# DavidLBick/espnet-1

Measured on AMD Instinct MI355X. Metric: utterances/sec + step-time, Conformer-L T=1000 batch=32 @1/2/4/8 GPU, higher is better.
Workload: dtype bf16; 1 GPU; C3 Conformer-L (12x512, 8 heads, ff 2048, cnn 31) + 6-layer Transformer decoder, hybrid CTC/att 0.3/0.7, lsm 0.1, V=5000, T=1000 frames x 80, L=40, dropout 0.1, Adam+WarmupLR+clip 5; global_batch=32, seq_len=1000, parallelism=dp1

## Files before the change

espnet-1_amd/csrc/gemm.hip:

```cpp

#include "gemm_kern.h"
#include <cstdio>
#include <cstdlib>

namespace {
__global__ void splitk_reduce(GemmP p) {
  const long MN = (long)p.M * p.N;
  const int z = blockIdx.y;
  const int zb = z / p.nh, zh = z % p.nh;
  const float* base = p.ws + (long)z * p.splitk * MN;
  const bool vec = p.vec_c && (p.N % 4 == 0);
  const EpiK ek = make_epik(p);
  const long n4 = vec ? MN / 4 : MN;
  for (long i = blockIdx.x * (long)blockDim.x + threadIdx.x; i < n4; i += (long)gridDim.x * blockDim.x) {
    if (vec) {
      float4 a = make_float4(0.f, 0.f, 0.f, 0.f);
      int s = 0;
      for (; s + 8 <= p.splitk; s += 8) {
        float4 b[8];
#pragma unroll
        for (int j = 0; j < 8; ++j) b[j] = *(const float4*)(base + (long)(s + j) * MN + i * 4);
#pragma unroll
        for (int j = 0; j < 8; ++j) { a.x += b[j].x; a.y += b[j].y; a.z += b[j].z; a.w += b[j].w; }
      }
// ... 80 lines not shown
  EA_LAUNCH_CHECK();
  return 0;
}

}

extern "C" int ea_gemm_set_pipeline(int stages) {
  EA_ENTRY();
  EA_CHECK_ARG(stages == 0 || stages == 2 || stages == 12);
  g_gemm_bm64 = stages < 10;
  g_gemm_stages = stages % 10;
  return 0;
}

namespace {
__global__ void probe_begin_kernel(unsigned long long* s) { s[0] = ~0ull; s[1] = 0ull; }
__global__ void probe_end_kernel(unsigned long long* s) {
  if (s[1] > s[0]) { s[2] += s[1] - s[0]; s[3] += 1ull; }
}
}

namespace {
__global__ void phase_stamp_kernel(unsigned long long* st, float* ring, int cap, int phase, const float* extra,
                                   const int* skip) {
  const unsigned long long now = __builtin_amdgcn_s_memrealtime();
  if (phase > 0) {
    const long slot = (long)(st[1] % (unsigned long long)cap);
    float dt = (float)((double)(now - st[0]) * 1e-8);
    if (phase == 3 && skip && skip[0]) dt = __builtin_nanf("");
    ring[slot * 4 + phase - 1] = dt;
    if (phase == 3) {
      ring[slot * 4 + 3] = extra ? extra[0] : 0.f;
      st[1] = st[1] + 1ull;
    }
  }
  st[0] = now;
}
}

extern "C" int ea_phase_stamp(unsigned long long* state, float* ring, int cap, int phase, const float* extra,
                              void* stream) {
  EA_ENTRY();
  EA_CHECK_ARG(state != nullptr && ring != nullptr && cap > 0 && phase >= 0 && phase <= 3);
  hipLaunchKernelGGL(phase_stamp_kernel, dim3(1), dim3(1), 0, (hipStream_t)stream, state, ring, cap, phase, extra,
                     (const int*)nullptr);
  EA_LAUNCH_CHECK();
  return 0;
}

extern "C" int ea_phase_stamp_opt(unsigned long long* state, float* ring, int cap, int phase,
                                  const ea_opt_state* opt, void* stream) {
  EA_ENTRY();
  EA_CHECK_ARG(state != nullptr && ring != nullptr && cap > 0 && phase >= 0 && phase <= 3 && opt != nullptr);
  hipLaunchKernelGGL(phase_stamp_kernel, dim3(1), dim3(1), 0, (hipStream_t)stream, state, ring, cap, phase,
                     &opt->next_lr, &opt->skip);
  EA_LAUNCH_CHECK();
  return 0;
}

extern "C" int ea_gemm_set_diag(unsigned long long* buf) {
  EA_ENTRY();
  g_diag = buf;
  return 0;
}

extern "C" int ea_gemm_set_probe(unsigned long long* slots) {
  EA_ENTRY();
  g_probe = slots;
  return 0;
}

extern "C" int ea_probe_begin(unsigned long long* slots, void* stream) {
  EA_ENTRY();
  EA_CHECK_ARG(slots != nullptr);
  hipLaunchKernelGGL(probe_begin_kernel, dim3(1), dim3(1), 0, (hipStream_t)stream, slots);
  EA_LAUNCH_CHECK();
  return 0;
}

extern "C" int ea_probe_end(unsigned long long* slots, void* stream) {
  EA_ENTRY();
  EA_CHECK_ARG(slots != nullptr);
  hipLaunchKernelGGL(probe_end_kernel, dim3(1), dim3(1), 0, (hipStream_t)stream, slots);
  EA_LAUNCH_CHECK();
  return 0;
}

extern "C" int ea_gemm_set_pipe(int on) {
  EA_ENTRY();
  g_gemm_pipe = on;
  return 0;
}

extern "C" int ea_gemm_set_k128(int mode, int slots) {
  EA_ENTRY();
  EA_CHECK_ARG(mode >= 0 && mode <= 3 && (slots == 3 || slots == 4));
  g_gemm_k128 = mode;
  eag::g_k128_slots = slots;
  return 0;
}

extern "C" int ea_gemm_set_skinny(int max_m) {
  EA_ENTRY();
  EA_CHECK_ARG(max_m >= 0 && max_m <= 64);
  g_gemm_skinny = max_m;
  return 0;
}

extern "C" int ea_gemm_set_tile(int bm, int bn) {
  EA_ENTRY();
  EA_CHECK_ARG((bm == 0 && bn == 0) || (bm == 32 && bn == 128) || (bm == 64 && bn == 128) ||
               (bm == 128 && bn == 128) || (bm == 256 && bn == 256));
  g_force_bm = bm;
  g_force_bn = bn;
  return 0;
}

static int gemm_impl(int dtype, int a_kmajor, int b_kmajor, int M, int N, int K,
                     const void* A, long lda, long sAb, long sAh,
                     const void* B, long ldb, long sBb, long sBh,
                     int batch, int nh,
                     void* C, int c_dtype, long ldc, long sCb, long sCh,
                     const ea_epilogue* epi, float* workspace, long ws_elems, void* stream,
                     const ea_conv_geo* geo, const float* w1x = nullptr, int w1T = 0, int w1F = 0,
                     float* w1part = nullptr, const uint8_t* w1pos = nullptr) {
  EA_CHECK_ARG(epi != nullptr && M >= 0 && N >= 0 && K >= 0 && batch >= 1 && nh >= 1);
  EA_CHECK_ARG(dtype == EA_F32 || dtype == EA_BF16);
  if (M == 0 || N == 0) return 0;
  const int E = dtype == EA_BF16 ? 8 : 4;
  const int esz = dtype == EA_BF16 ? 2 : 4;
  (void)esz;
  if (epi->kind == EA_EPI_RESID) EA_CHECK_ARG(c_dtype == EA_F32);
  GemmP p{};
  p.M = M; p.N = N; p.K = K;
  p.A = A; p.lda = lda; p.sAb = sAb; p.sAh = sAh;
  p.B = B; p.ldb = ldb; p.sBb = sBb; p.sBh = sBh;
  p.nh = nh;
  p.C = C; p.c_dtype = c_dtype; p.ldc = ldc; p.sCb = sCb; p.sCh = sCh;
  p.epi = *epi;
  p.ws = workspace;
  p.salt = ea_g_rng_salt;
  p.stamp = g_probe;
  p.diag = g_diag;
  p.g = geo ? *geo : ea_conv_geo{};
  p.w1x = w1x; p.w1part = w1part; p.w1pos = w1pos; p.w1T = w1T; p.w1F = w1F;
  p.vec_a = (lda % E == 0 && sAb % E == 0 && sAh % E == 0 && ((uintptr_t)A % 16) == 0);
  p.vec_b = (ldb % E == 0 && sBb % E == 0 && sBh % E == 0 && ((uintptr_t)B % 16) == 0);
  {
    const int ce = c_dtype == EA_BF16 ? 2 : 4;
    bool vc = (N % 4 == 0) && ldc % 4 == 0 && sCb % 4 == 0 && sCh % 4 == 0 && ((uintptr_t)C % (4 * ce)) == 0;
    if (epi->bias) vc = vc && ((uintptr_t)epi->bias % 16) == 0;
    if (epi->aux) vc = vc && epi->ldaux % 4 == 0 && ((uintptr_t)epi->aux % (4 * (epi->aux_dtype == EA_BF16 ? 2 : 4))) == 0;
    if (epi->resid) vc = vc && epi->ldr % 4 == 0 && ((uintptr_t)epi->resid % 16) == 0;
    p.vec_c = vc;
    bool v8 = vc && N % 8 == 0 && ldc % 8 == 0 && sCb % 8 == 0 && sCh % 8 == 0 && ((uintptr_t)C % 16) == 0;
    if (epi->aux) v8 = v8 && epi->ldaux % 8 == 0 && ((uintptr_t)epi->aux % 16) == 0;
    if (epi->resid) v8 = v8 && epi->ldr % 8 == 0;
    p.vec8 = v8;
  }
  p.bm = 128; p.bn = 128;
  if (dtype == EA_BF16 && M <= g_gemm_skinny && a_kmajor && b_kmajor && !geo && !w1part &&
      batch * nh == 1 && K % 32 == 0 && K > 0 && p.vec_a && p.vec_b) {
    static const bool trace_s = std::getenv("EA_GEMM_TRACE") != nullptr;
    if (trace_s) std::fprintf(stderr, "[ea_gemm] M=%d N=%d K=%d skinny epi=%d\n", M, N, K, (int)epi->kind);
    return launch_skinny(p, (hipStream_t)stream);
  }
  const double a_ext = 2.0 * ((a_kmajor ? (double)M : (double)K) * lda);
  const double b_ext = 2.0 * ((b_kmajor ? (double)N : (double)K) * ldb);
  const bool lds_path = dtype == EA_BF16 && p.vec_a && p.vec_b && g_gemm_stages > 0 &&
                        a_ext < 4.0e9 && b_ext < 4.0e9;
  p.lds = lds_path;
  if (geo && geo->mode != 0) {
    if (!lds_path || K % 64 != 0 || geo->C % 64 != 0 || batch * nh != 1) return EA_ERR_BAD_ARG;
    if ((geo->mode == EA_CONV_WGRAD) == (a_kmajor != 0) || (geo->mode == EA_CONV_FWD) != (b_kmajor != 0))
      return EA_ERR_BAD_ARG;
    choose_tile(p, 0, 1);
    if (geo->mode == EA_CONV_WGRAD && !g_force_bm) { p.bm = 256; p.bn = 256; }
    if (w1part) {
      if (!g_gemm_pipe || !p.vec8) return EA_ERR_BAD_ARG;
      p.bm = 256; p.bn = 256;
    }
    if (p.bm != 256 || p.bn != 256) { p.bm = 128; p.bn = 128; }
  } else if (lds_path) {
    choose_tile(p, a_kmajor, (long)batch * nh);
  }
  bool k128 = false;
  if (g_gemm_k128 && lds_path && !geo && a_kmajor && b_kmajor && K % 64 == 0 && K > 0) {
    const long t128 = (long)ea_cdiv(M, 128) * ea_cdiv(N, 128) * batch * nh;
    const bool fits = g_gemm_k128 == 3 ||
                      (!g_force_bm && (p.bm == 64 || p.bm == 128) && p.bn == 128 && t128 >= 128 &&
                       (g_gemm_k128 == 2 || (t128 <= 256 && K >= 1024)));
    if (fits) { p.bm = 128; p.bn = 128; k128 = true; }
  }
  if (p.bm <= 64 && !a_kmajor) return EA_ERR_BAD_ARG;
  p.tiles_m = ea_cdiv(M, p.bm);
  p.tiles_n = ea_cdiv(N, p.bn);
  const int KT = dtype == EA_BF16 ? KCfg<bf16>::KT : KCfg<float>::KT;
  const int nz = batch * nh;
  int splitk = 1;
  const long tiles = max(1L, (long)p.tiles_m * p.tiles_n * nz * (p.bm * p.bn) / (128 * 128));
  if (geo && geo->mode == EA_CONV_WGRAD && p.bm == 256) {
    if (workspace) {
      splitk = max(1, 256 / (p.tiles_m * p.tiles_n));
      splitk = min(splitk, K / (4 * KT));
      while (splitk > 1 && (long)splitk * M * N > ws_elems) --splitk;
      splitk = max(splitk, 1);
    }
  } else if (!k128 && workspace && tiles < 200 && K >= 16 * KT && K >= 1024 && (long)p.tiles_m * p.tiles_n * nz < 128) {
    splitk = (int)((384 + tiles - 1) / tiles);
    splitk = min(splitk, K / (4 * KT));
    splitk = min(splitk, 16);
    while (splitk > 1 && (long)splitk * nz * M * N > ws_elems) --splitk;
    if (splitk < 1) splitk = 1;
  }
  int kchunk = K;
  if (splitk > 1) {
    kchunk = ea_cdiv(ea_cdiv(K, splitk), KT) * KT;
    splitk = ea_cdiv(K, kchunk);
  }
  p.splitk = splitk;
  p.kchunk = kchunk;
  static const bool trace = std::getenv("EA_GEMM_TRACE") != nullptr;
  if (trace)
    std::fprintf(stderr, "[ea_gemm] M=%d N=%d K=%d ak=%d bk=%d nz=%d tile=%dx%d%s splitk=%d epi=%d geo=%d lds=%d\n", M,
                 N, K, a_kmajor, b_kmajor, nz, p.bm, p.bn, k128 ? "k" : "", splitk, (int)epi->kind, geo ? geo->mode : 0,
                 (int)p.lds);
  hipStream_t st = (hipStream_t)stream;
  int rc = dtype == EA_BF16 ? launch<bf16>(p, a_kmajor, b_kmajor, nz, st, k128)
                            : launch<float>(p, a_kmajor, b_kmajor, nz, st);
  if (rc) return rc;
  if (splitk > 1) {
    const long MN = (long)M * N;
    dim3 grid(ea_grid_cap(ea_cdiv(MN / 4 + 1, 256), 2048), nz);
    hipLaunchKernelGGL(splitk_reduce, grid, dim3(256), 0, st, p);
    EA_LAUNCH_CHECK();
  }
  return 0;
}

extern "C" int ea_gemm(int dtype, int a_kmajor, int b_kmajor, int M, int N, int K,
                       const void* A, long lda, long sAb, long sAh,
                       const void* B, long ldb, long sBb, long sBh,
                       int batch, int nh,
                       void* C, int c_dtype, long ldc, long sCb, long sCh,
                       const ea_epilogue* epi, float* workspace, long ws_elems, void* stream) {
  EA_ENTRY();
  return gemm_impl(dtype, a_kmajor, b_kmajor, M, N, K, A, lda, sAb, sAh, B, ldb, sBb, sBh, batch, nh, C, c_dtype,
                   ldc, sCb, sCh, epi, workspace, ws_elems, stream, nullptr);
}

extern "C" int ea_gemm_ln(int M, int N, int K, const float* x, long ldx, const float* gamma, const float* beta,
                          float eps, const void* W, long ldw, void* C, int c_dtype, long ldc, const ea_epilogue* epi,
                          void* stream) {
  EA_ENTRY();
  EA_CHECK_ARG(epi != nullptr && M >= 0 && N >= 0 && K > 0 && K % 32 == 0 && K <= 32 * 8 * 8);
  EA_CHECK_ARG(x && gamma && beta && W && C && ldx >= K && ldw >= K && ldc >= N);
  EA_CHECK_ARG(ldx % 4 == 0 && ((uintptr_t)x % 16) == 0 && ldw % 8 == 0 && ((uintptr_t)W % 16) == 0 &&
               ((uintptr_t)gamma % 16) == 0 && ((uintptr_t)beta % 16) == 0);
  if (epi->kind == EA_EPI_RESID) EA_CHECK_ARG(c_dtype == EA_F32);
  if (M == 0 || N == 0) return 0;
  GemmP p{};
  p.M = M; p.N = N; p.K = K;
  p.A = x; p.lda = ldx;
  p.B = W; p.ldb = ldw;
  p.nh = 1; p.splitk = 1; p.kchunk = K;
  p.C = C; p.c_dtype = c_dtype; p.ldc = ldc;
  p.epi = *epi;
  p.salt = ea_g_rng_salt;
  const int ce = c_dtype == EA_BF16 ? 2 : 4;
  bool vc = (N % 4 == 0) && ldc % 4 == 0 && ((uintptr_t)C % (4 * ce)) == 0;
  if (epi->bias) vc = vc && ((uintptr_t)epi->bias % 16) == 0;
  if (epi->aux) vc = vc && epi->ldaux % 4 == 0 && ((uintptr_t)epi->aux % (4 * (epi->aux_dtype == EA_BF16 ? 2 : 4))) == 0;
  if (epi->resid) vc = vc && epi->ldr % 4 == 0 && ((uintptr_t)epi->resid % 16) == 0;
  p.vec_c = vc;
  return launch_skinny_ln(p, gamma, beta, eps, (hipStream_t)stream);
}

extern "C" int ea_gemm_conv(const ea_conv_geo* geo, int a_kmajor, int b_kmajor, int M, int N, int K,
                            const void* A, long lda, const void* B, long ldb, void* C, int c_dtype, long ldc,
                            const ea_epilogue* epi, float* workspace, long ws_elems, void* stream) {
  EA_ENTRY();
  EA_CHECK_ARG(geo != nullptr && geo->mode >= EA_CONV_FWD && geo->mode <= EA_CONV_WGRAD);
  return gemm_impl(EA_BF16, a_kmajor, b_kmajor, M, N, K, A, lda, 0, 0, B, ldb, 0, 0, 1, 1, C, c_dtype, ldc, 0, 0,
                   epi, workspace, ws_elems, stream, geo);
}

extern "C" int ea_gemm_conv_w1(const ea_conv_geo* geo, int M, int N, int K, const void* A, long lda, const void* B,
                               long ldb, const ea_epilogue* epi, const float* x, int T, int Fin, float* part,
                               void* stream) {
  EA_ENTRY();
  EA_CHECK_ARG(geo != nullptr && geo->mode == EA_CONV_DGRAD && x != nullptr && part != nullptr);
  EA_CHECK_ARG(epi != nullptr && epi->kind == EA_EPI_DACT && epi->act == EA_ACT_RELU && epi->aux != nullptr &&
               epi->aux_dtype == EA_BF16);
  EA_CHECK_ARG(T >= 3 && Fin >= 3 && M < (1 << 24));
  return gemm_impl(EA_BF16, 1, 0, M, N, K, A, lda, 0, 0, B, ldb, 0, 0, 1, 1, nullptr, EA_BF16, N, 0, 0, epi,
                   nullptr, 0, stream, geo, x, T, Fin, part);
}

extern "C" int ea_gemm_conv_w1b(const ea_conv_geo* geo, int M, int N, int K, const void* A, long lda, const void* B,
                                long ldb, const ea_epilogue* epi, const float* x, int T, int Fin, float* part,
                                const unsigned char* pos, void* stream) {
  EA_ENTRY();
  EA_CHECK_ARG(geo != nullptr && geo->mode == EA_CONV_DGRAD && x != nullptr && part != nullptr && pos != nullptr);
  EA_CHECK_ARG(epi != nullptr && epi->kind == EA_EPI_DACT && epi->act == EA_ACT_RELU && N % 8 == 0);
  EA_CHECK_ARG(T >= 3 && Fin >= 3 && M < (1 << 24));
  return gemm_impl(EA_BF16, 1, 0, M, N, K, A, lda, 0, 0, B, ldb, 0, 0, 1, 1, nullptr, EA_BF16, N, 0, 0, epi,
                   nullptr, 0, stream, geo, x, T, Fin, part, pos);
}


extern "C" int ea_gemm_conv_w1b_all(const ea_conv_geo* geo, int N, const void* A, long lda, const void* B, long ldb,
                                    const ea_epilogue* epi, const float* x, int T, int Fin, float* part,
                                    const unsigned char* pos, void* stream) {
  EA_ENTRY();
  EA_CHECK_ARG(geo != nullptr && geo->mode == EA_CONV_DGRAD && x != nullptr && part != nullptr && pos != nullptr);
  EA_CHECK_ARG(epi != nullptr && epi->kind == EA_EPI_DACT && epi->act == EA_ACT_RELU);
  EA_CHECK_ARG(N >= 8 && N % 8 == 0 && geo->C % 64 == 0 && T >= 3 && Fin >= 3 && g_gemm_pipe != 0);
  EA_CHECK_ARG(lda % 8 == 0 && ldb % 8 == 0 && ((uintptr_t)A % 16) == 0 && ((uintptr_t)B % 16) == 0);
  GemmP p{};
  p.N = N;
  p.A = A; p.lda = lda;
  p.B = B; p.ldb = ldb;
  p.nh = 1; p.splitk = 1;
  p.C = nullptr; p.c_dtype = EA_BF16; p.ldc = N;
  p.epi = *epi;
  p.salt = ea_g_rng_salt;
  p.stamp = g_probe;
  p.diag = g_diag;
  p.g = *geo;
  p.w1x = x; p.w1part = part; p.w1pos = pos; p.w1T = T; p.w1F = Fin;
  p.vec_a = p.vec_b = p.vec_c = p.vec8 = p.lds = 1;
  p.bm = p.bn = 256;
  p.tiles_n = ea_cdiv(N, 256);
  int items = 0, tiles = 0;
  for (int c = 0; c < 4; ++c) {
    const int a = c >> 1, e = c & 1;
    const long rows = (long)geo->B * geo->nI[a] * geo->nJ[e];
    EA_CHECK_ARG(rows < (1L << 24));
    if (rows == 0) continue;
    const int k = p.ncls++;
    p.cls_item0[k] = items;
    p.cls_M[k] = (int)rows;
    p.cls_K[k] = (a ? 1 : 2) * (e ? 1 : 2) * geo->C;
    p.cls_a[k] = a;
    p.cls_e[k] = e;
    p.cls_tile0[k] = tiles;
    p.cls_pos[k] = geo->plane[c] / geo->C * (N / 8);
    tiles += (int)ea_cdiv(rows, 256);
    items += (int)ea_cdiv(rows, 256) * p.tiles_n;
  }
  if (p.ncls == 0) return 0;
  p.cls_item0[p.ncls] = items;
  p.M = p.cls_M[0]; p.K = p.cls_K[0]; p.kchunk = p.K; p.tiles_m = ea_cdiv(p.M, 256);
  const int unit = 8 * p.tiles_n;
  const dim3 grid((unsigned)(ea_cdiv(items, unit) * unit));
  static const bool trace = std::getenv("EA_GEMM_TRACE") != nullptr;
  if (trace) std::fprintf(stderr, "[ea_gemm] conv dgrad x%d classes, %d tiles, grid %u\n", p.ncls, items, grid.x);
  return launch_pipe_conv(p, grid, (hipStream_t)stream);
}
```

espnet-1_amd/csrc/gemm_kern.h:

```cpp
#pragma once
#include "common.h"


namespace eag {

constexpr int BM = 128, BN = 128, NT = 256;
constexpr int TILE_BYTES = 16384;

template <typename T> struct KCfg;
template <> struct KCfg<bf16> { static constexpr int KT = 64, KS = 32, E = 8, NKS = 2; };
template <> struct KCfg<float> { static constexpr int KT = 32, KS = 4, E = 4, NKS = 8; };

struct GemmP {
  int M, N, K;
  const void* A; long lda, sAb, sAh;
  const void* B; long ldb, sBb, sBh;
  int nh, splitk, kchunk;
  void* C; int c_dtype; long ldc, sCb, sCh;
  ea_epilogue epi;
  float* ws;
  int tiles_m, tiles_n;
  int vec_a, vec_b;
  int vec_c;
  int vec8;
// ... 1109 lines not shown
    const int row = c >> 2, ch = c & 3;
    return row * 64 + ((ch ^ swz32(row)) << 4);
  } else {
    const int pnl = c >> 9, cj = c & 511, k = cj >> 4, ch = cj & 15;
    return pnl * 8192 + k * 256 + ((ch ^ swz_mn_bf16(k)) << 4);
  }
}

EA_DEV s16x4 tr_read_asm(const char* p) {
  s16x4 v;
  const uint32_t a = (uint32_t)(uintptr_t)(const __attribute__((address_space(3))) char*)p;
  asm volatile("ds_read_b64_tr_b16 %0, %1" : "=v"(v) : "v"(a) : "memory");
  return v;
}

template <bool KMAJ>
EA_DEV bf16x8 frag32(const char* img, int r, int lane) {
  if (KMAJ) {
    const int row = r + (lane & 15), ch = lane >> 4;
    return *(const bf16x8*)(img + row * 64 + ((ch ^ swz32(row)) << 4));
  }
  const char* pnl = img + (r >> 7) * 8192;
  const int i = lane & 15, q = i >> 2, pp = i & 3;
  const int col = (r & 127) + 4 * pp;
  const int ch = col >> 3, within = (col & 7) * 2;
  union { bf16x8 v; s16x4 h[2]; } out;
#pragma unroll
  for (int half = 0; half < 2; ++half) {
    const int row = 8 * (lane >> 4) + 4 * half + q;
    out.h[half] = tr_read_asm(pnl + row * 256 + ((ch ^ swz_mn_bf16(row)) << 4) + within);
  }
  return out.v;
}

template <int BT, int NS = 4>
struct PipeT {
  static constexpr int BK = 32, NSLOT = NS, NW = 8, NTT = 512;
  static constexpr int A_BYTES = BT * BK * 2, B_BYTES = BT * BK * 2, SLOT = A_BYTES + B_BYTES;
  static constexpr int RING = NSLOT * SLOT;
  static constexpr int MI = BT == 256 ? 8 : 2;
  static constexpr int EPI_BYTES = NW * (MI < 4 ? MI : 4) * 16 * EPI_LDT * 4;
  static constexpr int SMEM = RING > EPI_BYTES ? RING : EPI_BYTES;
  static constexpr int ACH = A_BYTES / (NTT * 16), BCH = B_BYTES / (NTT * 16);
  static constexpr int G = ACH + BCH;
  static constexpr int OCC = BT == 256 ? 1 : 2;
  static_assert(BT == 256 || BT == 128, "pipe tiles");
  static_assert(NS == 4, "ring depth: 4 slots (5- and 6/8-slot rings measured slower, round 3/4)");
  EA_DEV static int wm(int w) { return BT == 256 ? (w >> 2) * 128 : (w >> 2) * 64 + ((w >> 1) & 1) * 32; }
  EA_DEV static int wn(int w) { return BT == 256 ? (w & 3) * 64 : (w & 1) * 64; }
};

struct TileOv {
  int M, a, e;
  float* w1part;
  const uint8_t* w1pos;
};
EA_DEV TileOv tile_ov(const GemmP& p) { return TileOv{p.M, p.g.a, p.g.e, p.w1part, p.w1pos}; }

template <bool AK, bool BKM, int MODE = 0, int BT = 256, int NS = 4>
EA_DEV void pipe_tile(const GemmP& p, const TileOv& ov, char* smem, const bf16* A, const bf16* B, int m0, int n0, int kbeg,
                      int kend, f32x4 (&acc)[PipeT<BT, NS>::MI][4]) {
  static_assert(MODE == 0 || (MODE == EA_CONV_FWD && AK && BKM) || (MODE == EA_CONV_DGRAD && AK) ||
                (MODE == EA_CONV_WGRAD && !AK && !BKM), "conv gather layouts");
  static_assert(MODE == 0 || BT == 256, "conv gathers run on 256-wide tiles");
  using PC = PipeT<BT, NS>;
  constexpr int BK = PC::BK, NSLOT = PC::NSLOT, NW = PC::NW, NTT = PC::NTT, MI = PC::MI;
  constexpr int A_BYTES = PC::A_BYTES, B_BYTES = PC::B_BYTES, SLOT = PC::SLOT;
  constexpr int ACH = PC::ACH, BCH = PC::BCH, G = PC::G;
  const int tid = threadIdx.x, lane = tid & 63, w = tid >> 6;
  const int wm = PC::wm(w), wn = PC::wn(w);
  const int nsl = max(0, (kend - kbeg) / BK);
  const bool tail = kbeg + nsl * BK < kend;


  auto src = [&](long ld, int mn0, int MN, bool kmaj, int ci) -> uint32_t {
    if (kmaj) {
      const int row = ci >> 2, c = (ci & 3) ^ swz32(ci >> 2);
      return (uint32_t)(((long)min(mn0 + row, MN - 1) * ld + c * 8) * 2);
    }
    const int pnl = ci >> 9, cj = ci & 511, k = cj >> 4, c = (cj & 15) ^ swz_mn_bf16(k);
    return (uint32_t)(((long)k * ld + min((long)(mn0 + pnl * 128 + c * 8), (long)((MN - 1) & ~7))) * 2);
  };
  const char* abase = (const char*)(A + (AK ? (long)kbeg : (long)kbeg * p.lda));
  const char* bbase = (const char*)(B + (BKM ? (long)kbeg : (long)kbeg * p.ldb));
  uint32_t aoff[ACH], boff[BCH];
#pragma unroll
  for (int i = 0; i < ACH; ++i) aoff[i] = src(p.lda, m0, ov.M, AK, (i * NW + w) * 64 + lane);
#pragma unroll
  for (int i = 0; i < BCH; ++i) boff[i] = src(p.ldb, n0, p.N, BKM, (i * NW + w) * 64 + lane);
  const long astep = (AK ? BK : (long)BK * p.lda) * 2;
  const long bstep = (BKM ? BK : (long)BK * p.ldb) * 2;

  const int ksl0 = kbeg / BK;
  const int CS = MODE ? p.g.C / BK : 1;
  int gb[ACH], gt[ACH], gf[ACH], cur[ACH];
  if constexpr (MODE == EA_CONV_FWD || MODE == EA_CONV_DGRAD) {
    const int n2 = MODE == EA_CONV_FWD ? p.g.T2 : p.g.nI[ov.a];
    const int n3 = MODE == EA_CONV_FWD ? p.g.F2 : p.g.nJ[ov.e];
#pragma unroll
    for (int i = 0; i < ACH; ++i) {
      const int m = min(m0 + ((((i * NW + w) * 64 + lane)) >> 2), ov.M - 1);
      const int bt = fdiv(m, n3);
      gf[i] = m - bt * n3;
      gb[i] = fdiv(bt, n2);
      gt[i] = bt - gb[i] * n2;
      cur[i] = 0;
    }
  }
  auto a_tap = [&](int q) {
#pragma unroll
    for (int i = 0; i < ACH; ++i) {
      const int ci = (i * NW + w) * 64 + lane;
      const int cc = ((ci & 3) ^ swz32(ci >> 2)) * 8;
      if constexpr (MODE == EA_CONV_FWD) {
        const int kh = q / 3, kw = q - 3 * (q / 3);
        cur[i] = (int)x1p_row(p.g, gb[i], gt[i], gf[i], kh, kw) + cc;
      } else {
        int kh, kw;
        dgrad_tap2(ov.a, ov.e, q, kh, kw);
        const int t2 = gt[i] - (kh >> 1), f2 = gf[i] - (kw >> 1);
        cur[i] = (t2 >= 0 && t2 < p.g.T2 && f2 >= 0 && f2 < p.g.F2)
                     ? ((gb[i] * p.g.T2 + t2) * p.g.F2 + f2) * p.g.C + cc
                     : (int)p.g.zero + ((ci >> 2) & 63) * p.g.C + cc;
      }
    }
  };
  int wb[BCH], wt[BCH], wf[BCH], wpix[BCH], wbase[BCH], wnI[BCH], wnJ[BCH];
  if constexpr (MODE == EA_CONV_WGRAD) {
#pragma unroll
    for (int i = 0; i < BCH; ++i) {
      const int ci = (i * NW + w) * 64 + lane;
      const int pnl = ci >> 9, cj = ci & 511, k = cj >> 4, c = (cj & 15) ^ swz_mn_bf16(k);
      const int n = min(n0 + pnl * 128 + c * 8, p.N - 8);
      const int tap = n / p.g.C, cin = n - tap * p.g.C;
      const int kh = tap / 3, kw = tap - 3 * kh, a = kh & 1, e = kw & 1;
      wnI[i] = p.g.nI[a];
      wnJ[i] = p.g.nJ[e];
      wbase[i] = (int)p.g.plane[a * 2 + e] + ((kh >> 1) * wnJ[i] + (kw >> 1)) * p.g.C + cin;
      const int pix = ksl0 * BK + k;
      wpix[i] = pix;
      const int bt = fdiv(pix, p.g.F2);
      wf[i] = pix - bt * p.g.F2;
      wb[i] = fdiv(bt, p.g.T2);
      wt[i] = bt - wb[i] * p.g.T2;
    }
  }
  const int dF = BK % max(p.g.F2, 1), dT = BK / max(p.g.F2, 1);

  auto issue = [&](int sl) {
    char* base = smem + (sl % NSLOT) * SLOT;
    const char* ak = abase + sl * astep;
    const char* bk = bbase + sl * bstep;
    if constexpr (MODE == EA_CONV_FWD || MODE == EA_CONV_DGRAD) {
      const int ks = ksl0 + sl;
      int q, c0;
      bool newtap;
      if constexpr (MODE == EA_CONV_FWD) {
        const int cb = ks / 18, r = ks - 18 * cb;
        q = r >> 1;
        c0 = cb * 64 + (r & 1) * BK;
        newtap = (r & 1) == 0;
      } else {
        q = ks / CS;
        c0 = (ks - q * CS) * BK;
        newtap = c0 == 0;
      }
      if (newtap || sl == 0) a_tap(q);
#pragma unroll
      for (int i = 0; i < ACH; ++i)
        __builtin_amdgcn_global_load_lds((__attribute__((address_space(1))) void*)((const char*)A + (long)(cur[i] + c0) * 2),
                                         (__attribute__((address_space(3))) void*)(base + (i * NW + w) * 1024), 16, 0, 0);
      if constexpr (MODE == EA_CONV_DGRAD) {
        int kh, kw;
        dgrad_tap2(ov.a, ov.e, q, kh, kw);
        bk = BKM ? (const char*)(B + (long)(kh * 3 + kw) * p.g.C + c0)
                 : (const char*)(B + ((long)(kh * 3 + kw) * p.g.C + c0) * p.g.C);
      }
    } else {
#pragma unroll
      for (int i = 0; i < ACH; ++i)
        __builtin_amdgcn_global_load_lds((__attribute__((address_space(1))) void*)(ak + aoff[i]),
                                         (__attribute__((address_space(3))) void*)(base + (i * NW + w) * 1024), 16, 0, 0);
    }
    if constexpr (MODE == EA_CONV_WGRAD) {
#pragma unroll
      for (int i = 0; i < BCH; ++i) {
        const int off = wpix[i] < p.g.P ? wbase[i] + ((wb[i] * wnI[i] + wt[i]) * wnJ[i] + wf[i]) * p.g.C
                                        : (int)p.g.zero + (lane & 63) * p.g.C + (wbase[i] % p.g.C);
        __builtin_amdgcn_global_load_lds((__attribute__((address_space(1))) void*)((const char*)B + (long)off * 2),
                                         (__attribute__((address_space(3))) void*)(base + A_BYTES + (i * NW + w) * 1024),
                                         16, 0, 0);
        wpix[i] += BK;
        wf[i] += dF;
        wt[i] += dT;
        if (wf[i] >= p.g.F2) { wf[i] -= p.g.F2; ++wt[i]; }
        while (wt[i] >= p.g.T2) { wt[i] -= p.g.T2; ++wb[i]; }
      }
    } else {
#pragma unroll
      for (int i = 0; i < BCH; ++i)
        __builtin_amdgcn_global_load_lds((__attribute__((address_space(1))) void*)(bk + boff[i]),
                                         (__attribute__((address_space(3))) void*)(base + A_BYTES + (i * NW + w) * 1024),
                                         16, 0, 0);
    }
  };

  auto rd_b = [&](int sl, bf16x8 (&fb)[4]) {
    const char* lb = smem + (sl % NSLOT) * SLOT + A_BYTES;
#pragma unroll
    for (int j = 0; j < 4; ++j) fb[j] = frag32<BKM>(lb, wn + j * 16, lane);
  };
  auto rd_a = [&](int sl, bf16x8 (&fa)[MI]) {
    const char* la = smem + (sl % NSLOT) * SLOT;
#pragma unroll
    for (int i = 0; i < MI; ++i) fa[i] = frag32<AK>(la, wm + i * 16, lane);
  };

  const int g1 = w >> 2;
  const int npre = min(NSLOT - 1, nsl);
  for (int sl = 0; sl < npre; ++sl) issue(sl);
  wait_newer<G, NSLOT - 2>(npre - 1);
  lds_barrier();
  if (g1) lds_barrier();
  bf16x8 fa[MI], fb[4];
  for (int sl = 0; sl < nsl; ++sl) {
    __builtin_amdgcn_sched_barrier(0);
    rd_b(sl, fb);
    rd_a(sl, fa);
    if (sl + NSLOT - 1 < nsl) issue(sl + NSLOT - 1);
    wait_newer<G, NSLOT - 2>(min(NSLOT - 2, nsl - 2 - sl));
    if (!AK || !BKM) {
      asm volatile("s_waitcnt lgkmcnt(0)" ::: "memory");
      __builtin_amdgcn_sched_barrier(0);
    }
#pragma unroll
    for (int i = 0; i < MI; ++i) asm volatile("" ::"v"(fa[i]));
#pragma unroll
    for (int j = 0; j < 4; ++j) asm volatile("" ::"v"(fb[j]));
    __builtin_amdgcn_sched_barrier(0);
    lds_barrier();
    __builtin_amdgcn_sched_barrier(0);
    __builtin_amdgcn_s_setprio(1);
#pragma unroll
    for (int i = 0; i < MI; ++i)
#pragma unroll
      for (int j = 0; j < 4; ++j)
        acc[i][j] = __builtin_amdgcn_mfma_f32_16x16x32_bf16(fa[i], fb[j], acc[i][j], 0, 0, 0);
    __builtin_amdgcn_s_setprio(0);
    __builtin_amdgcn_sched_barrier(0);
    lds_barrier();
  }
  if (!g1) lds_barrier();
  if (tail) {
    constexpr int NCH = (A_BYTES + B_BYTES) / 16 / NTT;
    uint4 v[NCH];
    const int k0 = kbeg + nsl * BK;
#pragma unroll
    for (int i = 0; i < NCH; ++i) {
      const int c = tid + NTT * i;
      const bool isa = c < A_BYTES / 16;
      const int cc = isa ? c : c - A_BYTES / 16;
      const bool km = isa ? AK : BKM;
      const bf16* base = isa ? A : B;
      const long ld = isa ? p.lda : p.ldb;
      const int MN = isa ? ov.M : p.N, mn0 = isa ? m0 : n0;
      int mn, k;
      if (km) { mn = mn0 + (cc >> 2); k = k0 + (cc & 3) * 8; }
      else    { const int cj = cc & 511; k = k0 + (cj >> 4); mn = mn0 + (cc >> 9) * 128 + (cj & 15) * 8; }
      union { uint4 u; bf16 e[8]; } tv;
#pragma unroll
      for (int e = 0; e < 8; ++e) {
        const bool ok = km ? (mn < MN && k + e < kend) : (k < kend && mn + e < MN);
        tv.e[e] = ok ? (km ? base[(long)mn * ld + k + e] : base[(long)k * ld + mn + e]) : (bf16)0.f;
      }
      v[i] = tv.u;
    }
    __syncthreads();
#pragma unroll
    for (int i = 0; i < NCH; ++i) {
      const int c = tid + NTT * i;
      const bool isa = c < A_BYTES / 16;
      const int cc = isa ? c : c - A_BYTES / 16;
      const int off = isa ? (AK ? img32_off<true>(cc) : img32_off<false>(cc))
                          : A_BYTES + (BKM ? img32_off<true>(cc) : img32_off<false>(cc));
      *(uint4*)(smem + off) = v[i];
    }
    __syncthreads();
    rd_b(0, fb);
    rd_a(0, fa);
    asm volatile("s_waitcnt lgkmcnt(0)" ::: "memory");
    __builtin_amdgcn_sched_barrier(0);
#pragma unroll
    for (int i = 0; i < MI; ++i)
#pragma unroll
      for (int j = 0; j < 4; ++j)
        acc[i][j] = __builtin_amdgcn_mfma_f32_16x16x32_bf16(fa[i], fb[j], acc[i][j], 0, 0, 0);
  }

  __syncthreads();
}

constexpr int W1_TS = 264;
constexpr int W1_IMG = 16 * W1_TS * 2;
constexpr int W1_SMEM = PipeT<256>::SMEM + 2 * W1_IMG;

EA_DEV void w1_load_x(const GemmP& p, const TileOv& ov, int m0, float (&xv)[5]) {
  const int tid = threadIdx.x;
  const int row = tid >> 1, t0 = (tid & 1) * 5;
  const int m = m0 + row;
#pragma unroll
  for (int u = 0; u < 5; ++u) xv[u] = 0.f;
  if (m < ov.M) {
    const int a = ov.a, e = ov.e, nI = p.g.nI[a], nJ = p.g.nJ[e];
    const int bi = fdiv(m, nJ), j = m - bi * nJ;
    const int b = fdiv(bi, nI), i = bi - b * nI;
    const float* xp = p.w1x + ((long)b * p.w1T + 2 * (2 * i + a)) * p.w1F + 2 * (2 * j + e);
#pragma unroll
    for (int u = 0; u < 5; ++u) {
      const int t = t0 + u;
      xv[u] = t < 9 ? xp[(t / 3) * p.w1F + t % 3] : 1.f;
    }
  }
}
EA_DEV void w1_stage_x(char* xs, const float (&xv)[5]) {
  bf16* hi = (bf16*)xs;
  bf16* lo = (bf16*)(xs + W1_IMG);
  const int tid = threadIdx.x;
  const int row = tid >> 1, t0 = (tid & 1) * 5;
#pragma unroll
  for (int u = 0; u < 5; ++u) {
    const bf16 h = (bf16)xv[u];
    hi[(t0 + u) * W1_TS + row] = h;
    lo[(t0 + u) * W1_TS + row] = (bf16)(xv[u] - (float)h);
  }
  for (int q = tid; q < 6 * 256; q += 512) {
    const int t = 10 + (q >> 8), r = q & 255;
    hi[t * W1_TS + r] = (bf16)0.f;
    lo[t * W1_TS + r] = (bf16)0.f;
  }
}

EA_DEV void w1_epilogue(const GemmP& p, const TileOv& ov, char* smem, int m0, int n0, int wm, int wn, int lane, int w, int tm,
                        const f32x4 (&acc)[8][4]) {
  float* t = (float*)smem + w * 64 * EPI_LDT;
  const char* xh = smem + PipeT<256>::SMEM;
  const char* xl = xh + W1_IMG;
  const int g = lane >> 4, lc = lane & 15, rq = g * 4;
  const int lc8 = (lane & 7) * 8, rl = lane >> 3;
  const bf16* aux = (const bf16*)p.epi.aux;
  f32x4 out[4];
#pragma unroll
  for (int cb = 0; cb < 4; ++cb) out[cb] = (f32x4){0.f, 0.f, 0.f, 0.f};
#pragma unroll
  for (int ch = 0; ch < 2; ++ch) {
    if (ch) {
      __builtin_amdgcn_wave_barrier();
      asm volatile("" ::: "memory");
    }
#pragma unroll
    for (int i = 0; i < 4; ++i)
#pragma unroll
      for (int j = 0; j < 4; ++j)
#pragma unroll
        for (int rr = 0; rr < 4; ++rr) t[(i * 16 + rq + rr) * EPI_LDT + j * 16 + lc] = acc[ch * 4 + i][j][rr];
    __builtin_amdgcn_wave_barrier();
    asm volatile("" ::: "memory");
    const int rb = m0 + wm + ch * 64, col = n0 + wn + lc8;
    if (ov.w1pos) {
      uint32_t mb[8];
#pragma unroll
      for (int it = 0; it < 8; ++it)
        mb[it] = ov.w1pos[(long)min(rb + it * 8 + rl, ov.M - 1) * (p.N >> 3) + min(col, p.N - 8) / 8];
#pragma unroll
      for (int it = 0; it < 8; ++it) {
        float* tr = t + (it * 8 + rl) * EPI_LDT + lc8;
        float4 f0 = *(const float4*)tr, f1 = *(const float4*)(tr + 4);
        float v[8] = {f0.x, f0.y, f0.z, f0.w, f1.x, f1.y, f1.z, f1.w};
#pragma unroll
        for (int c = 0; c < 8; ++c) v[c] = (float)(bf16)(((mb[it] >> c) & 1u) ? v[c] : 0.f);
        *(float4*)tr = make_float4(v[0], v[1], v[2], v[3]);
        *(float4*)(tr + 4) = make_float4(v[4], v[5], v[6], v[7]);
      }
    } else {
#pragma unroll
      for (int h0 = 0; h0 < 8; h0 += 4) {
        float o[4][8];
#pragma unroll
        for (int it = 0; it < 4; ++it)
          ld8(aux, (long)min(rb + (h0 + it) * 8 + rl, ov.M - 1) * p.epi.ldaux + col, EA_BF16, o[it]);
#pragma unroll
        for (int it = 0; it < 4; ++it) {
          float* tr = t + ((h0 + it) * 8 + rl) * EPI_LDT + lc8;
          float4 f0 = *(const float4*)tr, f1 = *(const float4*)(tr + 4);
          float v[8] = {f0.x, f0.y, f0.z, f0.w, f1.x, f1.y, f1.z, f1.w};
#pragma unroll
          for (int c = 0; c < 8; ++c) v[c] = (float)(bf16)(o[it][c] > 0.f ? v[c] : 0.f);
          *(float4*)tr = make_float4(v[0], v[1], v[2], v[3]);
          *(float4*)(tr + 4) = make_float4(v[4], v[5], v[6], v[7]);
        }
      }
    }
    __builtin_amdgcn_wave_barrier();
    asm volatile("" ::: "memory");
#pragma unroll
    for (int ks = 0; ks < 2; ++ks) {
      const int pl = wm + ch * 64 + 32 * ks + 8 * g;
      const bf16x8 bh = *(const bf16x8*)(xh + (lc * W1_TS + pl) * 2);
      const bf16x8 bl = *(const bf16x8*)(xl + (lc * W1_TS + pl) * 2);
#pragma unroll
      for (int cb = 0; cb < 4; ++cb) {
        union { bf16x8 v; bf16 e[8]; } af;
#pragma unroll
        for (int e = 0; e < 8; ++e) af.e[e] = (bf16)t[(32 * ks + 8 * g + e) * EPI_LDT + 16 * cb + lc];
        out[cb] = __builtin_amdgcn_mfma_f32_16x16x32_bf16(af.v, bh, out[cb], 0, 0, 0);
        out[cb] = __builtin_amdgcn_mfma_f32_16x16x32_bf16(af.v, bl, out[cb], 0, 0, 0);
      }
    }
  }
  __syncthreads();
  float* cmb = (float*)smem;
  if (w >= 4) {
#pragma unroll
    for (int cb = 0; cb < 4; ++cb)
#pragma unroll
      for (int r = 0; r < 4; ++r) cmb[((w - 4) * 64 + 16 * cb + 4 * g + r) * 16 + lc] = out[cb][r];
  }
  __syncthreads();
  if (w < 4 && lc < 10) {
    float* prow = ov.w1part + (long)tm * 10 * p.N + (long)lc * p.N;
#pragma unroll
    for (int cb = 0; cb < 4; ++cb)
#pragma unroll
      for (int r = 0; r < 4; ++r) {
        const int co = n0 + wn + 16 * cb + 4 * g + r;
        if (co < p.N) prow[co] = out[cb][r] + cmb[(w * 64 + 16 * cb + 4 * g + r) * 16 + lc];
      }
  }
}

EA_DEV bool dgrad_class_item(const GemmP& p, TileOv& ov, TileIdx& ti) {
  const int bid = blockIdx.x, x = bid & 7, sq = bid >> 3, tn_n = p.tiles_n;
  const int item = ((sq / tn_n) * 8 + x) * tn_n + sq % tn_n;
  if (item >= p.cls_item0[p.ncls]) return false;
  int c = 0;
#pragma unroll
  for (int k = 1; k < 4; ++k) c += (k < p.ncls && item >= p.cls_item0[k]) ? 1 : 0;
  const int local = item - p.cls_item0[c];
  ov.M = p.cls_M[c];
  ov.a = p.cls_a[c];
  ov.e = p.cls_e[c];
  ov.w1part = p.w1part + (long)p.cls_tile0[c] * 10 * p.N;
  ov.w1pos = p.w1pos + p.cls_pos[c];
  ti.tm = local / tn_n;
  ti.tn = local % tn_n;
  ti.z = 0;
  ti.sk = p.cls_K[c];
  return true;
}

template <bool AK, bool BKM, int MODE, int BT, int NS>
EA_DEV void pipe_body(const GemmP& p, const TileOv& ov, const TileIdx& ti, char* smem) {
  using PC = PipeT<BT, NS>;
  constexpr int MI = PC::MI;
  const int tm = ti.tm, m0 = ti.tm * BT, n0 = ti.tn * BT;
  const bool cls = MODE == EA_CONV_DGRAD && p.ncls;
  const int z = ti.z, sk = cls ? 0 : ti.sk;
  const int zb = z / p.nh, zh = z % p.nh;
  const bf16* A = (const bf16*)p.A + zb * p.sAb + zh * p.sAh;
  const bf16* B = (const bf16*)p.B + zb * p.sBb + zh * p.sBh;
  const int kbeg = sk * p.kchunk;
  const int kend = cls ? ti.sk : min(p.K, kbeg + p.kchunk);
  const int tid = threadIdx.x, lane = tid & 63, w = tid >> 6;
  const int wm = PC::wm(w), wn = PC::wn(w);
  f32x4 acc[MI][4];
#pragma unroll
  for (int i = 0; i < MI; ++i)
#pragma unroll
    for (int j = 0; j < 4; ++j) acc[i][j] = (f32x4){0.f, 0.f, 0.f, 0.f};
  diag_stamp(p, 0);
  float w1x[5];
  if constexpr (MODE == EA_CONV_DGRAD) {
    if (p.w1part) w1_load_x(p, ov, m0, w1x);
  }
  pipe_tile<AK, BKM, MODE, BT, NS>(p, ov, smem, A, B, m0, n0, kbeg, kend, acc);
  diag_stamp(p, 1);
  if constexpr (MODE == EA_CONV_DGRAD) {
    if (p.w1part) {
      w1_stage_x(smem + PC::SMEM, w1x);
      __syncthreads();
      w1_epilogue(p, ov, smem, m0, n0, wm, wn, lane, w, tm, acc);
      return;
    }
  }
  const EpiK ek = make_epik(p);
  switch (p.splitk > 1 ? EA_EPI_STORE : p.epi.kind) {
    case EA_EPI_STORE: epi_wave<EA_EPI_STORE, MI, 4>(p, ek, smem, z, zb, zh, m0 + wm, n0 + wn, lane, w, acc, sk); break;
    case EA_EPI_ACT: epi_wave<EA_EPI_ACT, MI, 4>(p, ek, smem, z, zb, zh, m0 + wm, n0 + wn, lane, w, acc, sk); break;
    case EA_EPI_RESID: epi_wave<EA_EPI_RESID, MI, 4>(p, ek, smem, z, zb, zh, m0 + wm, n0 + wn, lane, w, acc, sk); break;
    default: epi_wave<EA_EPI_DACT, MI, 4>(p, ek, smem, z, zb, zh, m0 + wm, n0 + wn, lane, w, acc, sk); break;
  }
  if (p.diag) {
    __syncthreads();
    diag_stamp(p, 2);
  }
}

template <bool AK, bool BKM, int MODE = 0, int BT = 256, int NS = 4>
__global__ __launch_bounds__(512, (PipeT<BT, NS>::OCC)) void gemm_pipe(GemmP p) {
  using PC = PipeT<BT, NS>;
  __shared__ __attribute__((aligned(1024))) char smem[MODE == EA_CONV_DGRAD ? W1_SMEM : PC::SMEM];
  probe_start(p);
  TileOv ov = tile_ov(p);
  TileIdx ti;
  bool run = true;
  if (MODE == EA_CONV_DGRAD && p.ncls) run = dgrad_class_item(p, ov, ti);
  else ti = tile_index(p);
  if (run) pipe_body<AK, BKM, MODE, BT, NS>(p, ov, ti, smem);
  probe_end(p);
}

}
```

Baseline: 1900 utterances/s.

## Feed conv weight-grad epilogue MFMA directly from registers with prefetched ReLU mask bits

Rewrites the w1 (conv subsampling weight-gradient) epilogue so masked accumulators are converted to bf16 MFMA operands straight from registers, with no round trip through an LDS staging tile. The packed ReLU position bits are prefetched from global memory before the main K loop and staged in LDS afterward, overlapping their latency with compute. The x image is moved into the pipeline ring region, which can shrink the kernel's LDS footprint and may raise occupancy. Argument checks now require N%64 and 8-byte pos alignment, which narrows the shapes the path accepts.

```diff
diff --git a/espnet-1_amd/csrc/gemm.hip b/espnet-1_amd/csrc/gemm.hip
--- a/espnet-1_amd/csrc/gemm.hip
+++ b/espnet-1_amd/csrc/gemm.hip
@@ -406,7 +406,8 @@
                                 const unsigned char* pos, void* stream) {
   EA_ENTRY();
   EA_CHECK_ARG(geo != nullptr && geo->mode == EA_CONV_DGRAD && x != nullptr && part != nullptr && pos != nullptr);
-  EA_CHECK_ARG(epi != nullptr && epi->kind == EA_EPI_DACT && epi->act == EA_ACT_RELU && N % 8 == 0);
+  EA_CHECK_ARG(epi != nullptr && epi->kind == EA_EPI_DACT && epi->act == EA_ACT_RELU);
+  EA_CHECK_ARG(N % 64 == 0 && ((uintptr_t)pos % 8) == 0);
   EA_CHECK_ARG(T >= 3 && Fin >= 3 && M < (1 << 24));
   return gemm_impl(EA_BF16, 1, 0, M, N, K, A, lda, 0, 0, B, ldb, 0, 0, 1, 1, nullptr, EA_BF16, N, 0, 0, epi,
                    nullptr, 0, stream, geo, x, T, Fin, part, pos);
@@ -419,7 +420,8 @@
   EA_ENTRY();
   EA_CHECK_ARG(geo != nullptr && geo->mode == EA_CONV_DGRAD && x != nullptr && part != nullptr && pos != nullptr);
   EA_CHECK_ARG(epi != nullptr && epi->kind == EA_EPI_DACT && epi->act == EA_ACT_RELU);
-  EA_CHECK_ARG(N >= 8 && N % 8 == 0 && geo->C % 64 == 0 && T >= 3 && Fin >= 3 && g_gemm_pipe != 0);
+  EA_CHECK_ARG(N >= 64 && N % 64 == 0 && geo->C % 64 == 0 && T >= 3 && Fin >= 3 && g_gemm_pipe != 0);
+  EA_CHECK_ARG(((uintptr_t)pos % 8) == 0);
   EA_CHECK_ARG(lda % 8 == 0 && ldb % 8 == 0 && ((uintptr_t)A % 16) == 0 && ((uintptr_t)B % 16) == 0);
   GemmP p{};
   p.N = N;
diff --git a/espnet-1_amd/csrc/gemm_kern.h b/espnet-1_amd/csrc/gemm_kern.h
--- a/espnet-1_amd/csrc/gemm_kern.h
+++ b/espnet-1_amd/csrc/gemm_kern.h
@@ -1435,7 +1435,11 @@
 
 constexpr int W1_TS = 264;
 constexpr int W1_IMG = 16 * W1_TS * 2;
-constexpr int W1_SMEM = PipeT<256>::SMEM + 2 * W1_IMG;
+constexpr int W1_X_OFF = PipeT<256>::RING;
+constexpr int W1_CMB_BYTES = 4 * 64 * 16 * 4;
+constexpr int W1_BITS_OFF = W1_CMB_BYTES;
+constexpr int W1_SMEM = PipeT<256>::SMEM > W1_X_OFF + 2 * W1_IMG ? PipeT<256>::SMEM : W1_X_OFF + 2 * W1_IMG;
+static_assert(W1_BITS_OFF + 4 * 256 * 8 <= PipeT<256>::RING, "support words fit the ring");
 
 EA_DEV void w1_load_x(const GemmP& p, const TileOv& ov, int m0, float (&xv)[5]) {
   const int tid = threadIdx.x;
@@ -1473,81 +1477,78 @@
   }
 }
 
+EA_DEV void w1_load_bits(const GemmP& p, const TileOv& ov, int m0, int n0, uint2 (&bv)[2]) {
+  const int tid = threadIdx.x;
+  const int row = min(m0 + (tid >> 1), ov.M - 1), w0 = (tid & 1) * 2;
+  const uint8_t* src = ov.w1pos + (long)row * (p.N >> 3) + (n0 >> 3);
+#pragma unroll
+  for (int u = 0; u < 2; ++u)
+    bv[u] = n0 + (w0 + u) * 64 < p.N ? *(const uint2*)(src + (w0 + u) * 8) : make_uint2(0u, 0u);
+}
+EA_DEV void w1_stage_bits(char* bs, const uint2 (&bv)[2]) {
+  const int tid = threadIdx.x;
+  const int row = tid >> 1, w0 = (tid & 1) * 2;
+#pragma unroll
+  for (int u = 0; u < 2; ++u) *(uint2*)(bs + ((w0 + u) * 256 + row) * 8) = bv[u];
+}
 EA_DEV void w1_epilogue(const GemmP& p, const TileOv& ov, char* smem, int m0, int n0, int wm, int wn, int lane, int w, int tm,
                         const f32x4 (&acc)[8][4]) {
-  float* t = (float*)smem + w * 64 * EPI_LDT;
-  const char* xh = smem + PipeT<256>::SMEM;
+  const char* xh = smem + W1_X_OFF;
   const char* xl = xh + W1_IMG;
-  const int g = lane >> 4, lc = lane & 15, rq = g * 4;
-  const int lc8 = (lane & 7) * 8, rl = lane >> 3;
+  const int g = lane >> 4, lc = lane & 15;
   const bf16* aux = (const bf16*)p.epi.aux;
+  const bool live = n0 + wn < p.N;
+  const char* bits = smem + W1_BITS_OFF + ((wn >> 6) * 256 + wm + 4 * g) * 8;
   f32x4 out[4];
 #pragma unroll
   for (int cb = 0; cb < 4; ++cb) out[cb] = (f32x4){0.f, 0.f, 0.f, 0.f};
 #pragma unroll
-  for (int ch = 0; ch < 2; ++ch) {
-    if (ch) {
-      __builtin_amdgcn_wave_barrier();
-      asm volatile("" ::: "memory");
-    }
-#pragma unroll
-    for (int i = 0; i < 4; ++i)
-#pragma unroll
-      for (int j = 0; j < 4; ++j)
-#pragma unroll
-        for (int rr = 0; rr < 4; ++rr) t[(i * 16 + rq + rr) * EPI_LDT + j * 16 + lc] = acc[ch * 4 + i][j][rr];
-    __builtin_amdgcn_wave_barrier();
-    asm volatile("" ::: "memory");
-    const int rb = m0 + wm + ch * 64, col = n0 + wn + lc8;
-    if (ov.w1pos) {
-      uint32_t mb[8];
-#pragma unroll
-      for (int it = 0; it < 8; ++it)
-        mb[it] = ov.w1pos[(long)min(rb + it * 8 + rl, ov.M - 1) * (p.N >> 3) + min(col, p.N - 8) / 8];
-#pragma unroll
-      for (int it = 0; it < 8; ++it) {
-        float* tr = t + (it * 8 + rl) * EPI_LDT + lc8;
-        float4 f0 = *(const float4*)tr, f1 = *(const float4*)(tr + 4);
-        float v[8] = {f0.x, f0.y, f0.z, f0.w, f1.x, f1.y, f1.z, f1.w};
-#pragma unroll
-        for (int c = 0; c < 8; ++c) v[c] = (float)(bf16)(((mb[it] >> c) & 1u) ? v[c] : 0.f);
-        *(float4*)tr = make_float4(v[0], v[1], v[2], v[3]);
-        *(float4*)(tr + 4) = make_float4(v[4], v[5], v[6], v[7]);
-      }
-    } else {
-#pragma unroll
-      for (int h0 = 0; h0 < 8; h0 += 4) {
-        float o[4][8];
-#pragma unroll
-        for (int it = 0; it < 4; ++it)
-          ld8(aux, (long)min(rb + (h0 + it) * 8 + rl, ov.M - 1) * p.epi.ldaux + col, EA_BF16, o[it]);
-#pragma unroll
-        for (int it = 0; it < 4; ++it) {
-          float* tr = t + ((h0 + it) * 8 + rl) * EPI_LDT + lc8;
-          float4 f0 = *(const float4*)tr, f1 = *(const float4*)(tr + 4);
-          float v[8] = {f0.x, f0.y, f0.z, f0.w, f1.x, f1.y, f1.z, f1.w};
-#pragma unroll
-          for (int c = 0; c < 8; ++c) v[c] = (float)(bf16)(o[it][c] > 0.f ? v[c] : 0.f);
-          *(float4*)tr = make_float4(v[0], v[1], v[2], v[3]);
-          *(float4*)(tr + 4) = make_float4(v[4], v[5], v[6], v[7]);
+  for (int ip = 0; ip < 4; ++ip) {
+    typedef __attribute__((ext_vector_type(2))) float f32x2v;
+    typedef __attribute__((ext_vector_type(2))) __bf16 bf16x2v;
+    union { bf16x8 v; bf16x2v q[4]; } af[4];
+#pragma unroll
+    for (int h = 0; h < 2; ++h) {
+      const int i = 2 * ip + h;
+      uint32_t sw[4][2];
+      if (ov.w1pos) {
+        const uint4 q0 = *(const uint4*)(bits + i * 128), q1 = *(const uint4*)(bits + i * 128 + 16);
+        sw[0][0] = q0.x; sw[0][1] = q0.y; sw[1][0] = q0.z; sw[1][1] = q0.w;
+        sw[2][0] = q1.x; sw[2][1] = q1.y; sw[3][0] = q1.z; sw[3][1] = q1.w;
+      } else {
+#pragma unroll
+        for (int r = 0; r < 4; ++r) {
+          const bf16* ar = aux + (long)min(m0 + wm + 16 * i + 4 * g + r, ov.M - 1) * p.epi.ldaux + (live ? n0 + wn : 0) + lc;
+          float a[4];
+#pragma unroll
+          for (int j = 0; j < 4; ++j) a[j] = (float)ar[16 * j];
+          sw[r][0] = sw[r][1] = 0u;
+#pragma unroll
+          for (int j = 0; j < 4; ++j) sw[r][j >> 1] |= (live && a[j] > 0.f ? 1u : 0u) << (lc + 16 * (j & 1));
         }
       }
-    }
-    __builtin_amdgcn_wave_barrier();
-    asm volatile("" ::: "memory");
-#pragma unroll
-    for (int ks = 0; ks < 2; ++ks) {
-      const int pl = wm + ch * 64 + 32 * ks + 8 * g;
-      const bf16x8 bh = *(const bf16x8*)(xh + (lc * W1_TS + pl) * 2);
-      const bf16x8 bl = *(const bf16x8*)(xl + (lc * W1_TS + pl) * 2);
-#pragma unroll
-      for (int cb = 0; cb < 4; ++cb) {
-        union { bf16x8 v; bf16 e[8]; } af;
-#pragma unroll
-        for (int e = 0; e < 8; ++e) af.e[e] = (bf16)t[(32 * ks + 8 * g + e) * EPI_LDT + 16 * cb + lc];
-        out[cb] = __builtin_amdgcn_mfma_f32_16x16x32_bf16(af.v, bh, out[cb], 0, 0, 0);
-        out[cb] = __builtin_amdgcn_mfma_f32_16x16x32_bf16(af.v, bl, out[cb], 0, 0, 0);
-      }
+#pragma unroll
+      for (int j = 0; j < 4; ++j) {
+        float v[4];
+#pragma unroll
+        for (int r = 0; r < 4; ++r) {
+          const uint32_t keep = 0u - ((sw[r][j >> 1] >> (lc + 16 * (j & 1))) & 1u);
+          v[r] = __uint_as_float(__float_as_uint(acc[i][j][r]) & keep);
+        }
+        af[j].q[2 * h] = __builtin_convertvector((f32x2v){v[0], v[1]}, bf16x2v);
+        af[j].q[2 * h + 1] = __builtin_convertvector((f32x2v){v[2], v[3]}, bf16x2v);
+      }
+    }
+    const int pl = wm + 32 * ip + 4 * g;
+    union { bf16x8 v; uint2 d[2]; } bh, bl;
+    bh.d[0] = *(const uint2*)(xh + (lc * W1_TS + pl) * 2);
+    bh.d[1] = *(const uint2*)(xh + (lc * W1_TS + pl + 16) * 2);
+    bl.d[0] = *(const uint2*)(xl + (lc * W1_TS + pl) * 2);
+    bl.d[1] = *(const uint2*)(xl + (lc * W1_TS + pl + 16) * 2);
+#pragma unroll
+    for (int cb = 0; cb < 4; ++cb) {
+      out[cb] = __builtin_amdgcn_mfma_f32_16x16x32_bf16(af[cb].v, bh.v, out[cb], 0, 0, 0);
+      out[cb] = __builtin_amdgcn_mfma_f32_16x16x32_bf16(af[cb].v, bl.v, out[cb], 0, 0, 0);
     }
   }
   __syncthreads();
@@ -1612,16 +1613,25 @@
     for (int j = 0; j < 4; ++j) acc[i][j] = (f32x4){0.f, 0.f, 0.f, 0.f};
   diag_stamp(p, 0);
   float w1x[5];
+  uint2 w1b[2];
   if constexpr (MODE == EA_CONV_DGRAD) {
-    if (p.w1part) w1_load_x(p, ov, m0, w1x);
+    if (p.w1part) {
+      w1_load_x(p, ov, m0, w1x);
+      if (ov.w1pos) w1_load_bits(p, ov, m0, n0, w1b);
+    }
   }
   pipe_tile<AK, BKM, MODE, BT, NS>(p, ov, smem, A, B, m0, n0, kbeg, kend, acc);
   diag_stamp(p, 1);
   if constexpr (MODE == EA_CONV_DGRAD) {
     if (p.w1part) {
-      w1_stage_x(smem + PC::SMEM, w1x);
+      w1_stage_x(smem + W1_X_OFF, w1x);
+      if (ov.w1pos) w1_stage_bits(smem + W1_BITS_OFF, w1b);
       __syncthreads();
       w1_epilogue(p, ov, smem, m0, n0, wm, wn, lane, w, tm, acc);
+      if (p.diag) {
+        __syncthreads();
+        diag_stamp(p, 2);
+      }
       return;
     }
   }
```

New measurement: 1907 utterances/s (median of 3 runs). No clear change (+0.3%).
